# johannes-graeter/mono_lidar_depth

Measured on AMD Instinct MI355X. Metric: feature-depth associations/sec, higher is better.
Workload: dtype f64; 1 GPU; BASELINE config 2: 64x2048 cloud x 2000 features/frame, C0 parameters, 1024 HBM-resident frames/step/GPU; frame_slots_per_launch=1024, features_per_frame=2000, points_per_frame=131072, contexts=2, sequences=1, parallelism=sequence-per-gpu x1

## Files before the change

### mono_lidar_depth_amd/csrc/mld_api.hip

```cpp
#include <hip/hip_runtime.h>

#include <algorithm>

#include <cmath>
#include <cstdio>
#include <cstdlib>
#include <condition_variable>
#include <cstring>
#include <ctime>
#include <functional>
#include <limits>
#include <mutex>
#include <string>
#include <thread>
#include <vector>

#include "../../include/mld.h"
#include "mld_device.h"
#include "mld_kernels.hip"
#include "mld_ransac.hip"

using namespace mld;

namespace {
// ... 61 lines not shown
        }
    }
    void submit(std::function<int(std::string&)> j) {
        {
            std::lock_guard<std::mutex> lk(m);
            job = std::move(j);
            pending = true;
        }
        cv.notify_all();
    }
    int wait(std::string& e) {
        std::unique_lock<std::mutex> lk(m);
        cv.wait(lk, [&] { return !pending; });
        e = err;
        return rc;
    }
    void stop() {
        {
            std::lock_guard<std::mutex> lk(m);
            quit = true;
        }
        cv.notify_all();
        if (th.joinable()) th.join();
    }
};

struct ProjShare {
    hipStream_t stream = nullptr;
    int refs = 0;
};

struct mld_ctx {
    mld_params P{};
    mld_camera cam{};
    Calib calib{};
    int device = 0;
    hipStream_t stream = nullptr;
    bool own_stream = true;
    std::vector<Slot> slots;
    SlotDesc* d_slots = nullptr;
    unsigned char* dummy = nullptr;
    int32_t* queue_counts = nullptr;
    uint32_t* map_slab = nullptr;
    size_t map_stride = 0;
    int32_t* queue_slab = nullptr;
    uint32_t* bitmaps = nullptr;
    size_t bitmap_words = 0;
    std::vector<SlotDesc> h_descs;
    std::vector<SlotDesc> desc_stage;
    size_t lds_bytes = 0;
    size_t lds_fused = 0;
    size_t lds_classify = 0;
    bool classify_staged = true;
    int bm_ncol = 0, bm_ncolp = 0;
    bool force_thread_path = false;
    size_t proj_lds = 0;
    std::string err;
    int32_t* rs_flags = nullptr;
    int32_t* rs_cand = nullptr;
    int32_t* rs_block = nullptr;
    size_t rs_cap = 0;
    int32_t* rs_M = nullptr;
    int32_t* rs_S = nullptr;
    int32_t* rs_sample = nullptr;
    float* rs_sp = nullptr;
    int32_t* rs_counts = nullptr;
    size_t rs_counts_cap = 0;
    int32_t* rs_inl = nullptr;
    ransac::Result* rs_res = nullptr;
    unsigned char* sem_img = nullptr;
    size_t sem_img_cap = 0;
    float* sem_coeffs = nullptr;
    unsigned char* sem_groups = nullptr;
    size_t sem_groups_cap = 0;
    ransac::SemResult* sem_res = nullptr;
    double* trk_uv_cur = nullptr;
    double* trk_uv_last = nullptr;
    double* trk_depth_cur = nullptr;
    double* trk_depth_last = nullptr;
    int32_t* trk_type_cur = nullptr;
    int32_t* trk_type_last = nullptr;
    int32_t* trk_rank = nullptr;
    long long* trk_n_new = nullptr;
    size_t trk_cap = 0;
    unsigned char* trkb = nullptr;
    size_t trkb_cap = 0;
    int trkb_seqs = 0;
    TrkSeq* trkb_desc = nullptr;
    std::vector<TrkSeq> trkb_host;
    SlotDesc* d_sub = nullptr;
    int32_t* sub_counts = nullptr;
    size_t sub_cap = 0;
    std::vector<SlotDesc> h_sub;
    unsigned char* trk_stage = nullptr;
    size_t trk_stage_cap = 0;
    unsigned char* fr_host = nullptr;
    unsigned char* fr_dev = nullptr;
    size_t fr_cap = 0;
    unsigned char* fr_host_dev = nullptr;
    bool fr_zero_copy = true;
    bool fr_helper_on = true;
    hipEvent_t fr_ev[5] = {nullptr, nullptr, nullptr, nullptr, nullptr};
    double fr_us[10] = {0, 0, 0, 0, 0, 0, 0, 0, 0, 0};
    uint32_t* rsb_masks = nullptr;
    size_t rsb_mask_words = 0;
    PlaneDev* rsb_planes = nullptr;
// ... 186 lines not shown
    c.thrG_mode = P.treshold_depth_mode;
    c.thrG_min = (double)P.treshold_depth_min;
    c.thrG_max = (double)P.treshold_depth_max;
    c.thrL_en = P.treshold_depth_local_enabled;
    c.thrL_mode = P.treshold_depth_local_mode;
    c.thrL_type = P.treshold_depth_local_valuetype;
    c.thrL_val = P.treshold_depth_local_value;
    c.useTriMax = P.do_use_triangle_size_maximation;
    c.checkPlanar = P.do_check_triangleplanar_condition;
    c.planarThr = P.triangleplanar_crossnorm_treshold;
    c.orthThr = P.viewray_plane_orthoganality_treshold;
    c.cutBehind = P.do_use_cut_behind_camera;
    c.useRoad = P.do_use_ransac_plane;
    c.roadMode = P.plane_estimator_use_triangle_maximation ? 1 : 0;
    c.roadDistThr = P.ransac_plane_point_distance_treshold;
    c.roadDistThrF = (float)c.roadDistThr;
    c.padf2_ = 0.f;
    c.zxMinRel = P.plane_estimator_z_x_min_relation;
    c.usePCA = P.do_use_PCA;
    c.pcaAbsMin = P.pca_treshold_3_abs_min;
    c.pcaRelMax = P.pca_treshold_3_2_rel_max;
    c.pcaRelMin = P.pca_treshold_2_1_rel_min;
    ctx->lds_bytes = (size_t)cap * (3 * sizeof(double) + 2 * sizeof(int));
    c.threadPath = 1;
    c.xcdAware = 1;
    c.sortClasses = 4;
    c.k1max = 32;
    c.kMain = 24;
    c.kTotal = 40;
#ifdef MLD_AB_SWITCHES
    if (const char* e = std::getenv("MLD_FORCE_WAVE_PATH")) c.threadPath = (e[0] == '1') ? 0 : 1;
    if (const char* e = std::getenv("MLD_NO_XCD")) c.xcdAware = (e[0] == '1') ? 0 : 1;
    if (const char* e = std::getenv("MLD_SORT_CLASSES")) c.sortClasses = (e[0] == '4') ? 4 : 1;
    if (const char* e = std::getenv("MLD_FORCE_THREAD_PATH")) ctx->force_thread_path = e[0] == '1';
    if (const char* e = std::getenv("MLD_PROJ_LDS")) ctx->proj_lds = (size_t)std::atoll(e);
    if (const char* e = std::getenv("MLD_GATE")) ctx->gate_mode = e[0] != '0';
    if (const char* e = std::getenv("MLD_FRAME_COPY")) ctx->fr_zero_copy = e[0] != '1';
    if (const char* e = std::getenv("MLD_FRAME_HELPER")) ctx->fr_helper_on = e[0] != '0';
    if (const char* e = std::getenv("MLD_K1MAX")) c.k1max = std::min(std::max(std::atoi(e), 8), kK1MaxLimit);
    if (const char* e = std::getenv("MLD_KMAIN")) c.kMain = std::min(std::max(std::atoi(e), 8), c.k1max);
    if (std::getenv("MLD_K1MAX") || std::getenv("MLD_KMAIN")) c.kTotal = c.k1max + c.kMain;
    if (const char* e = std::getenv("MLD_KTOTAL")) c.kTotal = std::min(std::max(std::atoi(e), c.k1max), c.k1max + c.kMain);
#endif
    ctx->lds_fused = (size_t)c.kTotal * kWave * sizeof(uint32_t);
    ctx->bm_ncol = (ctx->cam.width + 31) / 32 + 1;
    ctx->bm_ncolp = ctx->bm_ncol | 1;
    const size_t cls_fixed = (size_t)(kClsBuckets + kClsThreads / kWave + 4) * sizeof(int);
    const size_t cls_bitmap = (size_t)c.bmStride * (size_t)ctx->bm_ncolp * sizeof(uint32_t);
    ctx->classify_staged = cls_fixed + cls_bitmap <= 128 * 1024;
#ifdef MLD_AB_SWITCHES
    if (const char* e = std::getenv("MLD_CLASSIFY_STAGED")) ctx->classify_staged = ctx->classify_staged && e[0] != '0';
#endif
    ctx->lds_classify = cls_fixed + (ctx->classify_staged ? cls_bitmap : 0);
}

hipStream_t projection_fork(mld_ctx* ctx, int& rc) {
    rc = MLD_OK;
    if (!ctx->proj_stream) return ctx->stream;
    hipError_t e = hipEventRecord(ctx->proj_fork, ctx->stream);
    if (e == hipSuccess) e = hipStreamWaitEvent(ctx->proj_stream, ctx->proj_fork, 0);
    if (e != hipSuccess) {
        ctx->err = std::string("projection stream (fork): ") + hipGetErrorString(e);
        rc = MLD_ERR_HIP;
    }
    return ctx->proj_stream;
}
int projection_join(mld_ctx* ctx) {
    if (!ctx->proj_stream) return MLD_OK;
    HIP_TRY(ctx, hipEventRecord(ctx->proj_join, ctx->proj_stream));
    HIP_TRY(ctx, hipStreamWaitEvent(ctx->stream, ctx->proj_join, 0));
    return MLD_OK;
}
struct ProjectionScope {
    mld_ctx* ctx;
    bool open = true;
    explicit ProjectionScope(mld_ctx* c) : ctx(c) {}
    int finish() {
        open = false;
        return projection_join(ctx);
    }
    ~ProjectionScope() {
        if (open && ctx->proj_stream) {
            const std::string keep = ctx->err;
            (void)projection_join(ctx);
            ctx->err = keep;
        }
    }
};

int enable_rs_batch_lds(mld_ctx* ctx, size_t lds) {
    static size_t enabled[64] = {};
    static std::mutex mtx;
    std::lock_guard<std::mutex> lk(mtx);
    size_t& cur = enabled[ctx->device & 63];
    if (lds <= cur) return MLD_OK;
    HIP_TRY(ctx, hipFuncSetAttribute(reinterpret_cast<const void*>(ransac::k_rs_batch),
                                     hipFuncAttributeMaxDynamicSharedMemorySize, (int)lds));
    cur = lds;
    return MLD_OK;
}

int check_slot(mld_ctx* ctx, int slot) {
    if (!ctx) return MLD_ERR_INVALID_ARG;
    if (slot < 0 || slot >= (int)ctx->slots.size()) return fail(ctx, MLD_ERR_INVALID_ARG, "slot out of range");
    return MLD_OK;
}
// ... 151 lines not shown
    }
    s.queues_in_slab = false;
    s.d.live_queue = nullptr;
    s.d.ovf_queue = nullptr;
    HIP_TRY(ctx, hipMalloc((void**)&s.d.ovf_queue, (size_t)F * 2 * sizeof(int32_t)));
    HIP_TRY(ctx, hipMalloc((void**)&s.d.live_queue, (size_t)F * sizeof(int32_t)));
    s.road_cap = (size_t)F;
    return MLD_OK;
}

int upload_descs(mld_ctx* ctx, int n_slots, hipStream_t st = nullptr, int first = 0, bool tags_in_descs = false);

int upload_small(mld_ctx* ctx, void* dst, const void* src, size_t bytes, hipStream_t st) {
    static_assert(sizeof(SlotDesc) % 4 == 0 && sizeof(TrkSeq) % 4 == 0 && sizeof(Calib) % 4 == 0, "k_upload moves 32-bit words");
    if (!bytes) return MLD_OK;
    if (bytes % 4) return fail(ctx, MLD_ERR_INVALID_ARG, "upload_small: size not a multiple of 4");
    if (bytes > ctx->up_gen_bytes) return fail(ctx, MLD_ERR_CAPACITY, "upload_small: table larger than the context's upload ring");
    const int g = ctx->up_next;
    if (ctx->up_busy[g]) HIP_TRY(ctx, hipEventSynchronize(ctx->up_ev[g]));
    if (!ctx->up_ev[g]) HIP_TRY(ctx, hipEventCreateWithFlags(&ctx->up_ev[g], hipEventDisableTiming));
    unsigned char* stage = ctx->up_base + (size_t)g * ctx->up_gen_bytes;
    std::memcpy(stage, src, bytes);
    const int words = (int)(bytes / 4);
    hipLaunchKernelGGL(mld::k_upload, dim3((unsigned)((words + 255) / 256)), dim3(256), 0, st, reinterpret_cast<uint32_t*>(dst),
                       reinterpret_cast<const uint32_t*>(stage), words);
    HIP_TRY(ctx, hipGetLastError());
    HIP_TRY(ctx, hipEventRecord(ctx->up_ev[g], st));
    ctx->up_busy[g] = true;
    ctx->up_next = (g + 1) % mld_ctx::kUpGens;
    return MLD_OK;
}

int launch_features(mld_ctx* ctx, int n_slots, int64_t max_F, bool single, int slot, const Calib* override_calib = nullptr,
                    const SlotDesc* group_descs = nullptr) {
    if (max_F <= 0) return MLD_OK;
    const SlotDesc* const descs = group_descs ? group_descs : ctx->d_slots;
    Calib calib = override_calib ? *override_calib : ctx->calib;
    const bool few = single && max_F <= 16384 && !ctx->force_thread_path;
    if (few) calib.threadPath = 0;
    const int per_slot = (int)((max_F + kWave - 1) / kWave);
    const uint32_t tag_all = (single || group_descs) ? 0u : common_tag(ctx, n_slots);
    const SlotDesc one = single ? ctx->slots[slot].d : SlotDesc{};
    const int use_single = single ? 1 : 0, ns = single ? 1 : n_slots;
    if (few) {
    } else {
        ScopedTimer ts(ctx, 5);
        auto kc = ctx->classify_staged ? mld::k_classify<true, kClsThreads, kClsKeep>
                                       : mld::k_classify<false, kClsThreads, kClsKeep>;
        const bool gate = ctx->gate_mode && ctx->release_waiter && !single;
        if (gate && !ctx->cls_done) {
            HIP_TRY(ctx, hipMalloc((void**)&ctx->cls_done, sizeof(uint32_t)));
            HIP_TRY(ctx, hipMemsetAsync(ctx->cls_done, 0, sizeof(uint32_t), ctx->stream));
        }
        hipLaunchKernelGGL(kc, dim3((unsigned)ns), dim3(kClsThreads), ctx->lds_classify, ctx->stream, descs, one,
                           use_single, calib, ctx->bm_ncol, ctx->bm_ncolp, gate ? ctx->cls_done : (uint32_t*)nullptr);
        if (gate) {
            mld_ctx* w = ctx->release_waiter;
            ctx->release_waiter = nullptr;
            w->waiting_on = nullptr;
            ctx->cls_target += (uint32_t)ns;
            if (w->gate_src && w->gate_src != ctx && w->gate_src->gate_waiter == w) w->gate_src->gate_waiter = nullptr;
            if (ctx->gate_waiter && ctx->gate_waiter != w) {
                ctx->gate_waiter->gate_counter = nullptr;
                ctx->gate_waiter->order_wait_pending = false;
                ctx->gate_waiter->gate_src = nullptr;
            }
            w->gate_counter = ctx->cls_done;
            w->gate_target = ctx->cls_target;
            w->order_wait_pending = true;
            w->gate_src = ctx;
            ctx->gate_waiter = w;
        }
    }
    if (ctx->release_waiter) {
        mld_ctx* w = ctx->release_waiter;
        ctx->release_waiter = nullptr;
        w->waiting_on = nullptr;
        HIP_TRY(ctx, hipEventRecord(w->order_ev, ctx->stream));
        if (w->gate_src && w->gate_src->gate_waiter == w) w->gate_src->gate_waiter = nullptr;
        w->gate_src = nullptr;
        w->gate_counter = nullptr;
        w->order_wait_pending = true;
    }
    int rc_up = MLD_OK;
    const Calib* d_calib = ctx->d_calib;
    {
        Calib want = calib;
        want.threadPath = ctx->calib.threadPath;
        const int which = std::memcmp(&want, &ctx->calib, sizeof(Calib)) == 0 ? 0 : 1;
        if (std::memcmp(&want, &ctx->calib_uploaded[which], sizeof(Calib)) != 0) {
            int rc_c = upload_small(ctx, ctx->d_calib + which, &want, sizeof(Calib), ctx->stream);
            if (rc_c) return rc_c;
            ctx->calib_uploaded[which] = want;
        }
        d_calib = ctx->d_calib + which;
    }
    if (calib.threadPath) {
        ScopedTimer tm(ctx, 1);
        int dense = (calib.k1max > 32 || calib.kMain > 24) ? ((ctx->shared_arg & 1) ? 1 : 2) : 0;
#ifdef MLD_AB_SWITCHES
        if (const char* e = std::getenv("MLD_FORCE_DENSE")) dense = std::min(std::max(std::atoi(e), 0), 2);
#endif
        auto kf = dense == 2 ? (calib.roadMode ? mld::k_feature_fused<1, 2> : mld::k_feature_fused<0, 2>)
                  : dense == 1 ? (calib.roadMode ? mld::k_feature_fused<1, 1> : mld::k_feature_fused<0, 1>)
                               : (calib.roadMode ? mld::k_feature_fused<1, 0> : mld::k_feature_fused<0, 0>);
        if (single && (rc_up = upload_descs(ctx, 1, nullptr, slot, true))) return rc_up;
        hipLaunchKernelGGL(kf, dim3((unsigned)per_slot * (unsigned)ns), dim3(kWave), ctx->lds_fused + ctx->lds_fused_pad, ctx->stream,
                           descs + (single ? slot : 0), d_calib, ns, per_slot);
    }
    {
        ScopedTimer tm(ctx, 3);
        const int chunk = few ? (int)std::min<int64_t>(8, std::max<int64_t>(1, (max_F + 8191) / 8192)) : 8;
        const int want = (int)((max_F + chunk - 1) / chunk);
// ... 169 lines not shown
        if (hipStreamCreateWithFlags(&fresh, hipStreamNonBlocking) != hipSuccess) break;
        rejected.push_back(ctx->stream);
        ctx->stream = fresh;
    }
    for (hipStream_t r : rejected) (void)hipStreamDestroy(r);
    g_live.push_back(ctx);
}
}

mld_ctx* mld_create(const mld_params* params, const mld_camera* camera, const double T_cam_lidar[12], int device,
                    int max_frames, int64_t max_points, int64_t max_features, int* status_out) {
    auto bail = [&](int code, const std::string& msg) -> mld_ctx* {
        g_create_error = msg;
        if (status_out) *status_out = code;
        return nullptr;
    };
    if (status_out) *status_out = MLD_OK;
    if (!params || !camera || !T_cam_lidar) return bail(MLD_ERR_INVALID_ARG, "null argument");
    if (max_frames < 1) return bail(MLD_ERR_INVALID_ARG, "max_frames must be >= 1");
    if (camera->width < 1 || camera->height < 1) return bail(MLD_ERR_INVALID_ARG, "bad image size");
    if (camera->width > 65535 || camera->height > 65535 || (int64_t)camera->width * camera->height > (int64_t)1 << 30)
        return bail(MLD_ERR_CAPACITY, "image larger than 65535 pixels on a side or 2^30 pixels in all");
    if (!std::isfinite(camera->focal_length) || camera->focal_length == 0.0 || !std::isfinite(camera->principal_point_x) ||
        !std::isfinite(camera->principal_point_y))
        return bail(MLD_ERR_INVALID_ARG, "bad camera intrinsics");
    for (int t = 0; t < 12; t++)
        if (!std::isfinite(T_cam_lidar[t])) return bail(MLD_ERR_INVALID_ARG, "non-finite lidar->camera transform");
    if (max_points > kMaxPoints) return bail(MLD_ERR_CAPACITY, "max_points exceeds 8 388 607");
    std::string why;
    int v = validate_params(*params, why);
    if (v != MLD_OK) return bail(v, why);

    int ndev = 0;
    hipError_t e = hipGetDeviceCount(&ndev);
    if (e != hipSuccess || ndev < 1)
        return bail(MLD_ERR_HIP, std::string("no HIP device available (") + hipGetErrorString(e) +
                                     "): the DepthEstimator path has no CPU fallback");
    if (device < 0 || device >= ndev) return bail(MLD_ERR_INVALID_ARG, "device index out of range");

    mld_ctx* ctx = new mld_ctx();
    ctx->P = *params;
    ctx->cam = *camera;
    ctx->device = device;
    build_calib(ctx, T_cam_lidar);
    auto hip_bail = [&](hipError_t err, const char* what) -> mld_ctx* {
        std::string m = std::string(what) + ": " + hipGetErrorString(err);
        mld_destroy(ctx);
        return bail(MLD_ERR_HIP, m);
    };
    if ((e = hipSetDevice(device)) != hipSuccess) return hip_bail(e, "hipSetDevice");
    hipDeviceProp_t prop;
    if ((e = hipGetDeviceProperties(&prop, device)) != hipSuccess) return hip_bail(e, "hipGetDeviceProperties");
    ctx->lds_per_cu = (size_t)prop.maxSharedMemoryPerMultiProcessor;
    if (ctx->lds_bytes > (size_t)prop.sharedMemPerBlock) {
        mld_destroy(ctx);
        return bail(MLD_ERR_CAPACITY, "search window too large for the LDS-staged neighbour list");
    }
    if ((e = hipStreamCreateWithFlags(&ctx->stream, hipStreamNonBlocking)) != hipSuccess)
        return hip_bail(e, "hipStreamCreate");
    separate_stream_from_live_contexts(ctx);
    if (ctx->lds_bytes > 48 * 1024) {
        e = hipFuncSetAttribute(reinterpret_cast<const void*>(mld::k_feature_wave<true>), hipFuncAttributeMaxDynamicSharedMemorySize,
                                (int)ctx->lds_bytes);
        if (e == hipSuccess)
            e = hipFuncSetAttribute(reinterpret_cast<const void*>(mld::k_feature_wave<false>),
                                    hipFuncAttributeMaxDynamicSharedMemorySize, (int)ctx->lds_bytes);
        if (e != hipSuccess) return hip_bail(e, "hipFuncSetAttribute(k_feature_wave)");
    }
    if (ctx->lds_classify > 48 * 1024) {
        e = hipFuncSetAttribute(reinterpret_cast<const void*>(mld::k_classify<true, kClsThreads, kClsKeep>),
                                hipFuncAttributeMaxDynamicSharedMemorySize, (int)ctx->lds_classify);

        if (e != hipSuccess) return hip_bail(e, "hipFuncSetAttribute(k_classify)");
    }
    if (ctx->lds_fused > 48 * 1024) {
        const void* fused[] = {reinterpret_cast<const void*>(mld::k_feature_fused<0, 0>),
                               reinterpret_cast<const void*>(mld::k_feature_fused<1, 0>),
                               reinterpret_cast<const void*>(mld::k_feature_fused<0, 1>),
                               reinterpret_cast<const void*>(mld::k_feature_fused<1, 1>),
                               reinterpret_cast<const void*>(mld::k_feature_fused<0, 2>),
                               reinterpret_cast<const void*>(mld::k_feature_fused<1, 2>)};
        for (const void* f : fused) {
            e = hipFuncSetAttribute(f, hipFuncAttributeMaxDynamicSharedMemorySize, (int)ctx->lds_fused);
            if (e != hipSuccess) return hip_bail(e, "hipFuncSetAttribute(k_feature_fused)");
        }
    }
    ctx->slots.resize(max_frames);
    ctx->h_descs.resize(max_frames);
    if ((e = hipMalloc((void**)&ctx->d_slots, sizeof(SlotDesc) * max_frames)) != hipSuccess)
        return hip_bail(e, "hipMalloc(slots)");
    if ((e = hipMalloc((void**)&ctx->dummy, 256)) != hipSuccess) return hip_bail(e, "hipMalloc(dummy)");
    if ((e = hipMalloc((void**)&ctx->d_calib, 2 * sizeof(Calib))) != hipSuccess) return hip_bail(e, "hipMalloc(calib)");
    std::memset(ctx->calib_uploaded, 0xFF, sizeof(ctx->calib_uploaded));
    constexpr size_t kMaxGroupDescs = 256;
    static_assert(kMaxGroupDescs <= 512, "the group descriptors of a launch set must fit one generation of the upload ring");
    static_assert(sizeof(TrkSeq) <= 2 * sizeof(SlotDesc), "a sequence's TrkSeq must fit the ring share of its two slots");
    const size_t up_descs = max_frames >= 2 ? std::max<size_t>((size_t)max_frames, 512) : 1;
    ctx->up_gen_bytes = (std::max(sizeof(SlotDesc) * up_descs, sizeof(Calib)) + 4095) / 4096 * 4096;
    if ((e = hipHostMalloc((void**)&ctx->up_base, ctx->up_gen_bytes * mld_ctx::kUpGens, hipHostMallocDefault)) != hipSuccess)
        return hip_bail(e, "hipHostMalloc(upload ring)");
    if ((e = hipMemsetAsync(ctx->dummy, 0, 256, ctx->stream)) != hipSuccess) return hip_bail(e, "hipMemset(dummy)");
    size_t cells = (size_t)camera->width * camera->height + kMapPadCells;
    ctx->bitmap_words = (size_t)ctx->calib.bmStride * (size_t)((camera->width + 31) / 32 + 1) + 4;
    const size_t cnt_words = 2 * (size_t)max_frames;
    if ((e = hipMalloc((void**)&ctx->queue_counts, (cnt_words + ctx->bitmap_words * (size_t)max_frames) * sizeof(uint32_t))) != hipSuccess)
        return hip_bail(e, "hipMalloc(bitmaps)");
    ctx->bitmaps = reinterpret_cast<uint32_t*>(ctx->queue_counts) + cnt_words;
    if ((e = hipMemsetAsync(ctx->queue_counts, 0, cnt_words * sizeof(uint32_t), ctx->stream)) != hipSuccess)
        return hip_bail(e, "hipMemset(counters)");
    for (size_t si = 0; si < ctx->slots.size(); si++) ctx->slots[si].d.bitmap = ctx->bitmaps + si * ctx->bitmap_words;
    for (size_t si = 0; si < ctx->slots.size(); si++) {
        ctx->slots[si].d.live_count = ctx->queue_counts + si;
        ctx->slots[si].d.ovf_count = ctx->queue_counts + (size_t)max_frames + si;
    }
    const size_t map_stride = (cells + 63) & ~(size_t)63;
    ctx->map_stride = map_stride;
    if ((e = hipMalloc((void**)&ctx->map_slab, map_stride * (size_t)max_frames * sizeof(uint32_t))) != hipSuccess)
        return hip_bail(e, "hipMalloc(maps)");
    if ((e = hipMemsetAsync(ctx->map_slab, 0, map_stride * (size_t)max_frames * sizeof(uint32_t), ctx->stream)) != hipSuccess)
        return hip_bail(e, "hipMemset(maps)");
    const size_t qF = max_features > 0 ? (((size_t)max_features + 63) & ~(size_t)63) : 0;
    const size_t q_stride = qF * 3;
    if (qF && (e = hipMalloc((void**)&ctx->queue_slab, q_stride * (size_t)max_frames * sizeof(int32_t))) != hipSuccess)
        return hip_bail(e, "hipMalloc(queues)");
    for (size_t si = 0; si < ctx->slots.size(); si++) {
        Slot& s = ctx->slots[si];
// ... 1745 lines not shown
```

### mono_lidar_depth_amd/csrc/mld_kernels.hip

```cpp
#include "mld_device.h"
#include "../../include/mld.h"
#include "mld_diag.h"

namespace mld {

#define GPTR(T, p) ((const T __attribute__((address_space(1)))*)(p))
#define GPTRW(T, p) ((T __attribute__((address_space(1)))*)(p))
#define CPTR(T, p) ((const T __attribute__((address_space(4)))*)(p))
typedef float f32x4 __attribute__((ext_vector_type(4)));
typedef uint32_t u32x4u __attribute__((ext_vector_type(4), aligned(4)));

__device__ __forceinline__ int prefix_count(unsigned long long m) {
    return (int)__builtin_amdgcn_mbcnt_hi((unsigned)(m >> 32), __builtin_amdgcn_mbcnt_lo((unsigned)m, 0u));
}
__device__ __forceinline__ int uniform(int v) { return __builtin_amdgcn_readfirstlane(v); }
__device__ __forceinline__ bool wave_any(bool p) { return __builtin_amdgcn_ballot_w64(p) != 0ull; }
__device__ __forceinline__ double readlane_f64(double v, int lane) {
    int lo = __double2loint(v), hi = __double2hiint(v);
    lo = __builtin_amdgcn_readlane(lo, lane);
    hi = __builtin_amdgcn_readlane(hi, lane);
    return __hiloint2double(hi, lo);
}
template <int CTRL, int ROW_MASK>
__device__ __forceinline__ int dpp_self(int v) {
// ... 2045 lines not shown
                }
            const double mx = sx / (double)n, my = sy / (double)n, mz = sz / (double)n;
            double c0 = 0, c1 = 0, c2 = 0, c3 = 0, c4 = 0, c5 = 0;
            for (int e = 0; e < nmax; e++)
                if (e < n) {
                    V3 p = cam_point(c, s, LST(e));
                    double dx = p.x - mx, dy = p.y - my, dz = p.z - mz;
                    c0 += dx * dx;
                    c1 += dx * dy;
                    c2 += dx * dz;
                    c3 += dy * dy;
                    c4 += dy * dz;
                    c5 += dz * dz;
                }
            r[0] = mx; r[1] = my; r[2] = mz;
            r[3] = c0; r[4] = c1; r[5] = c2; r[6] = c3; r[7] = c4; r[8] = c5;
        } else if (live) {
            V3 p0 = cam_point(c, s, LST(0)), p1 = cam_point(c, s, LST(1)), p2 = cam_point(c, s, LST(2));
            r[0] = p0.x; r[1] = p0.y; r[2] = p0.z;
            r[3] = p1.x; r[4] = p1.y; r[5] = p1.z;
            r[6] = p2.x; r[7] = p2.y; r[8] = p2.z;
        }
    }
    r[9] = minZ;
    r[10] = maxZ;
    ST_USE_F64(r[0]);
    ST_USE_F64(r[8]);
    ST_MARK(10);
    if (live) finish_main(c, pca, myu, myv, r, mytype, mydepth);
    ST_USE_F64(mydepth);
    ST_MARK(11);
}

template <int DENSE>
__device__ __forceinline__ void main_after_scan(const Calib& c, const SlotRef& s, uint32_t* lst, const int lane,
                                                const int lcap, const int k, bool live, const double myu, const double myv,
                                                int& mytype, double& mydepth, bool& overflow ST_ARG) {
    int ks;
    double minZ, maxZ;
    const int kmax0 = uniform(wave_max_i32(live ? k : 0));
    if (DENSE && kmax0 > kZcDefault && (kmax0 <= kZcMid || DENSE == 1))
        main_hist<DENSE ? kZcMid : kZcDefault>(c, s, lst, lane, lcap, k, live, mytype, ks, minZ, maxZ ST_PASS);
    else if (DENSE == 2 && kmax0 > kZcMid)
        main_hist<DENSE == 2 ? kZcDense : kZcDefault>(c, s, lst, lane, lcap, k, live, mytype, ks, minZ, maxZ ST_PASS);
    else if (DENSE == 0 && kmax0 <= kZcTiny)
        main_hist<DENSE == 0 ? kZcTiny : kZcDefault>(c, s, lst, lane, lcap, k, live, mytype, ks, minZ, maxZ ST_PASS);
    else if (DENSE == 0 && kmax0 <= kZcShort)
        main_hist<DENSE == 0 ? kZcShort : kZcDefault>(c, s, lst, lane, lcap, k, live, mytype, ks, minZ, maxZ ST_PASS);
    else
        main_hist<kZcDefault>(c, s, lst, lane, lcap, k, live, mytype, ks, minZ, maxZ ST_PASS);
    main_tail<DENSE>(c, s, lst, lane, lcap, ks, live, minZ, maxZ, myu, myv, mytype, mydepth, overflow ST_PASS);
}

template <bool DIRECT>
__global__ __launch_bounds__(kWave) void k_feature_wave(const SlotDesc* __restrict__ slots, SlotDesc single, int use_single,
                                                        const Calib* __restrict__ calib, int n_slots, int per_slot,
                                                        uint32_t tag_all, int chunk) {
    constexpr int direct = DIRECT ? 1 : 0;
    const Calib& c = *calib;
    extern __shared__ __align__(16) unsigned char smem[];
    int slot, j;
    decode_block((int)blockIdx.x, c.xcdAware ? n_slots : -n_slots, per_slot, slot, j);
    SlotDesc s = use_single ? single : slots[slot];
    apply_plane_dev(s);
    if (tag_all) s.tag = tag_all;
    int count;
    if (direct) {
        long long Fn = s.F;
        if (s.F_dev) {
            long long fd = *GPTR(long long, s.F_dev) - s.F_dev_off;
            fd = fd < 0 ? 0 : fd;
            Fn = fd < Fn ? fd : Fn;
        }
        count = (int)Fn;
    } else {
        if (!s.ovf_count) return;
        count = *GPTR(int32_t, s.ovf_count);
    }
    const int lane = threadIdx.x;
    auto pass = [&](const int e0) {
        bool active = lane < chunk && e0 + lane < count;
        long long f = 0;
        int code = 0;
        double myu = 0, myv = 0;
        if (active && direct) {
            f = e0 + lane;
            code = -1;
            const auto* q = GPTR(double, s.uv) + 2 * f;
            myu = q[0];
            myv = q[1];
            int x0, y0, nx, ny;
            if (window_bounds(c, myu, myv, c.halfX1, c.halfY1, x0, y0, nx, ny) && nx <= 32) {
                const auto* bm = GPTR(uint32_t, s.bitmap) + (size_t)(x0 >> 5) * (size_t)c.bmStride;
                const uint32_t sh = (uint32_t)(x0 & 31);
                const uint32_t colmask = (nx >= 32) ? ~0u : ((1u << nx) - 1u);
                int k1 = 0;
                for (int r = 0; r < ny; r++) {
                    const uint32_t lo = bm[y0 + r], hi = bm[c.bmStride + y0 + r];
                    k1 += __popc(__builtin_amdgcn_alignbit(hi, lo, sh) & colmask);
                }
                if ((unsigned)k1 < c.countMin) {
                    GPTRW(double, s.depth)[f] = -1.0;
                    if (s.type) GPTRW(int32_t, s.type)[f] = MLD_RadiusSearchInsufficientPoints;
                    active = false;
                }
            } else if (nx <= 32) {
                if (0u < c.countMin) {
                    GPTRW(double, s.depth)[f] = -1.0;
                    if (s.type) GPTRW(int32_t, s.type)[f] = MLD_RadiusSearchInsufficientPoints;
                    active = false;
                }
            }
        } else if (active) {
            f = (long long)GPTR(int32_t, s.ovf_queue)[2 * (size_t)(e0 + lane)];
            code = GPTR(int32_t, s.ovf_queue)[2 * (size_t)(e0 + lane) + 1];
            const auto* q = GPTR(double, s.uv) + 2 * f;
            myu = q[0];
            myv = q[1];
        }
        int mytype = code < 0 ? (int)MLD_Unspecified : code;
        double mydepth = -1.0;
        const unsigned long long all = __ballot(active);
        const unsigned long long full = __ballot(active && code < 0);
        double corners[9];
        bool has_corners = false;
        ST_BEGIN(1);
        wave_path(c, s, smem, lane, all, myu, myv, mytype, mydepth, full, corners, has_corners ST_PASS);
        if (active) {
            GPTRW(double, s.depth)[f] = mydepth;
            if (s.type) GPTRW(int32_t, s.type)[f] = mytype;
            if (s.corners && has_corners) {
#pragma unroll
                for (int t = 0; t < 9; t++) GPTRW(double, s.corners)[9 * f + t] = corners[t];
            }
        }
        ST_MARK(12);
        ST_END();
    };
    if (DIRECT) {
        if (j * chunk < count) pass(j * chunk);
    } else {
        for (int e0 = j * chunk; e0 < count; e0 += per_slot * chunk) pass(e0);
    }
}


__device__ __forceinline__ bool window_bounds(const Calib& c, double u, double v, double halfX, double halfY, int& x0,
                                              int& y0, int& nx, int& ny) {
    x0 = 0;
    y0 = 0;
    nx = 0;
    ny = 0;
    if (!(isfinite(u) && isfinite(v))) return false;
    double a;
    a = u - halfX;
    const double left = (a < 0.) ? 0. : a;
    a = u + halfX;
    const double right = ((double)(c.W - 1) < a) ? (double)(c.W - 1) : a;
    a = v - halfY;
    const double top = (a < 0.) ? 0. : a;
    a = v + halfY;
    const double bottom = ((double)(c.H - 1) < a) ? (double)(c.H - 1) : a;
    const int xa = (int)left, ya = (int)top, xb = (int)right, yb = (int)bottom;
    const int wx = xb - xa + 1, wy = yb - ya + 1;
    if (wx <= 0 || wy <= 0 || xa < 0 || ya < 0 || xb >= c.W || yb >= c.H) return false;
    x0 = xa;
    y0 = ya;
    nx = wx;
    ny = wy;
    return true;
}

constexpr int kClsThreads = 1024;
constexpr int kClsBuckets = 1024;
constexpr int kClsKeep = 2;
enum : int { CLS_DEAD = -1, CLS_OVF = -2, CLS_NONE = -3 };

template <bool STAGED, int kClsThreads, int kClsKeep>
__global__ __launch_bounds__(kClsThreads) void k_classify(const SlotDesc* __restrict__ slots, SlotDesc single,
                                                          int use_single, Calib c, int ncol, int ncolp,
                                                          uint32_t* __restrict__ done) {
    extern __shared__ __align__(16) unsigned char smem[];
    int* hist = reinterpret_cast<int*>(smem);
    int* wsum = hist + kClsBuckets;
    int* ctr = wsum + kClsThreads / kWave;
    uint32_t* lbm = reinterpret_cast<uint32_t*>(ctr + 4);
    SlotDesc s = use_single ? single : slots[blockIdx.x];
    apply_plane_dev(s);
    long long Fn = s.F;
    if (s.F_dev) {
        long long fd = *GPTR(long long, s.F_dev) - s.F_dev_off;
        fd = fd < 0 ? 0 : fd;
        Fn = fd < Fn ? fd : Fn;
    }
    const int tid = threadIdx.x, lane = tid & (kWave - 1), wave = tid >> 6;
// ... 105 lines not shown
                fu[q] = uv[2 * i];
                fv[q] = uv[2 * i + 1];
            }
        }
#pragma unroll
        for (int q = 0; q < kClsKeep; q++) {
            const long long i = tid + (long long)q * kClsThreads;
            kept[q] = (i < Fn) ? classify(fu[q], fv[q]) : (int)CLS_NONE;
            if (kept[q] >= 0) atomicAdd(&hist[kept[q]], 1);
            if (i < Fn) settle(i, kept[q]);
        }
    }
    for (long long i = tid + (long long)kClsKeep * kClsThreads; i < Fn; i += kClsThreads) {
        const int cls = classify(uv[2 * i], uv[2 * i + 1]);
        if (cls >= 0) atomicAdd(&hist[cls], 1);
        settle(i, cls);
    }
    __syncthreads();
    constexpr int kPer = kClsBuckets / kClsThreads;
    static_assert(kPer >= 1 && kPer * kClsThreads == kClsBuckets, "bucket count must be a multiple of the block size");
    int loc[kPer], sum = 0;
#pragma unroll
    for (int q = 0; q < kPer; q++) {
        loc[q] = hist[tid * kPer + q];
        sum += loc[q];
    }
    int incl = sum;
#pragma unroll
    for (int d = 1; d < kWave; d <<= 1) {
        const int t = __shfl_up(incl, d);
        if (lane >= d) incl += t;
    }
    if (lane == kWave - 1) wsum[wave] = incl;
    __syncthreads();
    int base = incl - sum;
    for (int q = 0; q < wave; q++) base += wsum[q];
    if (tid == kClsThreads - 1) {
        *GPTRW(int32_t, s.live_count) = base + sum;
        *GPTRW(int32_t, s.ovf_count) = ctr[0];
    }
#pragma unroll
    for (int q = 0; q < kPer; q++) {
        hist[tid * kPer + q] = base;
        base += loc[q];
    }
    __syncthreads();
    auto* live = GPTRW(int32_t, s.live_queue);
#pragma unroll
    for (int q = 0; q < kClsKeep; q++)
        if (kept[q] >= 0) live[atomicAdd(&hist[kept[q]], 1)] = (int32_t)(tid + q * kClsThreads);
    for (long long i = tid + (long long)kClsKeep * kClsThreads; i < Fn; i += kClsThreads) {
        const int cls = classify(uv[2 * i], uv[2 * i + 1]);
        if (cls >= 0) live[atomicAdd(&hist[cls], 1)] = (int32_t)i;
    }
}

__global__ __launch_bounds__(kWave) void k_gate(const uint32_t* __restrict__ counter, uint32_t target, int max_polls) {
    if (threadIdx.x != 0) return;
    for (int i = 0; i < max_polls; i++) {
        const uint32_t v = __hip_atomic_load(GPTR(uint32_t, counter), __ATOMIC_RELAXED, __HIP_MEMORY_SCOPE_AGENT);
        if ((int32_t)(v - target) >= 0) break;
        __builtin_amdgcn_s_sleep(32);
    }
}

__global__ __launch_bounds__(kWave) void k_probe_wait(const uint32_t* flag, uint32_t* result, int max_polls) {
    if (threadIdx.x != 0) return;
    uint32_t seen = 2u;
    for (int i = 0; i < max_polls; i++) {
        if (__hip_atomic_load(flag, __ATOMIC_RELAXED, __HIP_MEMORY_SCOPE_SYSTEM) != 0u) {
            seen = 1u;
            break;
        }
        __builtin_amdgcn_s_sleep(32);
    }
    __hip_atomic_store(result, seen, __ATOMIC_RELAXED, __HIP_MEMORY_SCOPE_SYSTEM);
}
__global__ void k_probe_set(uint32_t* flag) {
    if (threadIdx.x == 0 && blockIdx.x == 0) __hip_atomic_store(flag, 1u, __ATOMIC_RELAXED, __HIP_MEMORY_SCOPE_SYSTEM);
}

__global__ __launch_bounds__(256) void k_upload(uint32_t* __restrict__ dst, const uint32_t* __restrict__ src_host, int n_words) {
    const int i = blockIdx.x * 256 + threadIdx.x;
    if (i < n_words) dst[i] = __builtin_nontemporal_load(src_host + i);
}

#ifndef MLD_KEY_BATCH_F
#define MLD_KEY_BATCH_F 8
#endif
constexpr int kKeyBatchF = MLD_KEY_BATCH_F;
#ifndef MLD_DENSE_BATCH_MUL
#define MLD_DENSE_BATCH_MUL 2
#endif
constexpr int kDenseBatchMul = MLD_DENSE_BATCH_MUL;

template <int KB>
__device__ __forceinline__ int scan_window_flagged(const Calib& c, const SlotRef& s, int x0, int y0, int nx, int ny,
                                                   int xn0, int yn0, int nxn, int nyn, uint32_t* lst,
                                                   int lane, int& kflag, uint32_t& states, int& nbase, int& nroom ST_ARG) {
    const int nymax = uniform(wave_max_i32(ny));
    const auto* bm = GPTR(uint32_t, s.g.bitmap);
    const uint32_t colmask = (nx >= 32) ? ~0u : ((1u << nx) - 1u);
    const uint32_t nmask = (nxn > 0) ? (((nxn >= 32) ? ~0u : ((1u << nxn) - 1u)) << (xn0 - x0)) : 0u;
    int k = 0, kf = 0;
    const auto* col0 = bm + (size_t)(x0 >> 5) * (size_t)c.bmStride + (size_t)y0;
    const auto* col1 = col0 + c.bmStride;
// ... 448 lines not shown
```

Baseline: 2.833 billion feature-depth associations/s.

## Add persistent prefetching classify kernel and deal overflow work across waves

Adds k_classify_resident, a grid-limited persistent classify kernel. Each block loops over frame slots and prefetches the next slot's bitmap and uv data into registers while finishing the current one. It is only used when MLD_CLASSIFY_GRID is set, because the default grid value of -1 disables it. Separately, the overflow pass of k_feature_wave now spreads overflow entries across all waves with a stride instead of giving each wave a contiguous chunk. This balances lightly loaded slots at the cost of less coalesced queue reads.

```diff
diff --git a/mono_lidar_depth_amd/csrc/mld_api.hip b/mono_lidar_depth_amd/csrc/mld_api.hip
--- a/mono_lidar_depth_amd/csrc/mld_api.hip
+++ b/mono_lidar_depth_amd/csrc/mld_api.hip
@@ -137,6 +137,9 @@
     size_t lds_fused = 0;
     size_t lds_classify = 0;
     bool classify_staged = true;
+    size_t lds_classify_res = 0;
+    int cls_grid = kClsGridDefault;
+    int cu_count = 0;
     int bm_ncol = 0, bm_ncolp = 0;
     bool force_thread_path = false;
     size_t proj_lds = 0;
@@ -429,6 +432,7 @@
     if (const char* e = std::getenv("MLD_CLASSIFY_STAGED")) ctx->classify_staged = ctx->classify_staged && e[0] != '0';
 #endif
     ctx->lds_classify = cls_fixed + (ctx->classify_staged ? cls_bitmap : 0);
+    ctx->lds_classify_res = std::max(ctx->lds_classify, kClsResidentLds);
 }
 
 hipStream_t projection_fork(mld_ctx* ctx, int& rc) {
@@ -686,13 +690,20 @@
             HIP_TRY(ctx, hipMalloc((void**)&ctx->cls_done, sizeof(uint32_t)));
             HIP_TRY(ctx, hipMemsetAsync(ctx->cls_done, 0, sizeof(uint32_t), ctx->stream));
         }
-        hipLaunchKernelGGL(kc, dim3((unsigned)ns), dim3(kClsThreads), ctx->lds_classify, ctx->stream, descs, one,
-                           use_single, calib, ctx->bm_ncol, ctx->bm_ncolp, gate ? ctx->cls_done : (uint32_t*)nullptr);
+        const bool resident = !single && ctx->classify_staged && ctx->cls_grid >= 0 && ctx->cu_count > 0;
+        const int grid = !resident ? ns : std::min(ns, ctx->cls_grid > 0 ? ctx->cls_grid : ctx->cu_count);
+        if (resident)
+            hipLaunchKernelGGL(mld::k_classify_resident, dim3((unsigned)grid), dim3(kClsThreads), ctx->lds_classify_res,
+                               ctx->stream, descs, calib, ctx->bm_ncol, ctx->bm_ncolp, ns,
+                               gate ? ctx->cls_done : (uint32_t*)nullptr);
+        else
+            hipLaunchKernelGGL(kc, dim3((unsigned)ns), dim3(kClsThreads), ctx->lds_classify, ctx->stream, descs, one,
+                               use_single, calib, ctx->bm_ncol, ctx->bm_ncolp, gate ? ctx->cls_done : (uint32_t*)nullptr);
         if (gate) {
             mld_ctx* w = ctx->release_waiter;
             ctx->release_waiter = nullptr;
             w->waiting_on = nullptr;
-            ctx->cls_target += (uint32_t)ns;
+            ctx->cls_target += (uint32_t)grid;
             if (w->gate_src && w->gate_src != ctx && w->gate_src->gate_waiter == w) w->gate_src->gate_waiter = nullptr;
             if (ctx->gate_waiter && ctx->gate_waiter != w) {
                 ctx->gate_waiter->gate_counter = nullptr;
@@ -968,6 +979,8 @@
     hipDeviceProp_t prop;
     if ((e = hipGetDeviceProperties(&prop, device)) != hipSuccess) return hip_bail(e, "hipGetDeviceProperties");
     ctx->lds_per_cu = (size_t)prop.maxSharedMemoryPerMultiProcessor;
+    ctx->cu_count = prop.multiProcessorCount;
+    if (const char* e = std::getenv("MLD_CLASSIFY_GRID")) ctx->cls_grid = std::max(std::atoi(e), -1);
     if (ctx->lds_bytes > (size_t)prop.sharedMemPerBlock) {
         mld_destroy(ctx);
         return bail(MLD_ERR_CAPACITY, "search window too large for the LDS-staged neighbour list");
@@ -988,6 +1001,12 @@
                                 hipFuncAttributeMaxDynamicSharedMemorySize, (int)ctx->lds_classify);
 
         if (e != hipSuccess) return hip_bail(e, "hipFuncSetAttribute(k_classify)");
+    }
+    if (!ctx->classify_staged || ctx->lds_classify_res > ctx->lds_per_cu) ctx->cls_grid = -1;
+    if (ctx->cls_grid >= 0) {
+        e = hipFuncSetAttribute(reinterpret_cast<const void*>(mld::k_classify_resident),
+                                hipFuncAttributeMaxDynamicSharedMemorySize, (int)ctx->lds_classify_res);
+        if (e != hipSuccess) return hip_bail(e, "hipFuncSetAttribute(k_classify_resident)");
     }
     if (ctx->lds_fused > 48 * 1024) {
         const void* fused[] = {reinterpret_cast<const void*>(mld::k_feature_fused<0, 0>),
diff --git a/mono_lidar_depth_amd/csrc/mld_kernels.hip b/mono_lidar_depth_amd/csrc/mld_kernels.hip
--- a/mono_lidar_depth_amd/csrc/mld_kernels.hip
+++ b/mono_lidar_depth_amd/csrc/mld_kernels.hip
@@ -2121,6 +2121,10 @@
     main_tail<DENSE>(c, s, lst, lane, lcap, ks, live, minZ, maxZ, myu, myv, mytype, mydepth, overflow ST_PASS);
 }
 
+#ifndef MLD_WAVE_DEAL
+#define MLD_WAVE_DEAL 1
+#endif
+constexpr bool kWaveDeal = MLD_WAVE_DEAL != 0;
 template <bool DIRECT>
 __global__ __launch_bounds__(kWave) void k_feature_wave(const SlotDesc* __restrict__ slots, SlotDesc single, int use_single,
                                                         const Calib* __restrict__ calib, int n_slots, int per_slot,
@@ -2147,13 +2151,14 @@
         count = *GPTR(int32_t, s.ovf_count);
     }
     const int lane = threadIdx.x;
-    auto pass = [&](const int e0) {
-        bool active = lane < chunk && e0 + lane < count;
+    auto pass = [&](const int e0, const int estride) {
+        const int e = e0 + lane * estride;
+        bool active = lane < chunk && e < count;
         long long f = 0;
         int code = 0;
         double myu = 0, myv = 0;
         if (active && direct) {
-            f = e0 + lane;
+            f = e;
             code = -1;
             const auto* q = GPTR(double, s.uv) + 2 * f;
             myu = q[0];
@@ -2181,8 +2186,8 @@
                 }
             }
         } else if (active) {
-            f = (long long)GPTR(int32_t, s.ovf_queue)[2 * (size_t)(e0 + lane)];
-            code = GPTR(int32_t, s.ovf_queue)[2 * (size_t)(e0 + lane) + 1];
+            f = (long long)GPTR(int32_t, s.ovf_queue)[2 * (size_t)e];
+            code = GPTR(int32_t, s.ovf_queue)[2 * (size_t)e + 1];
             const auto* q = GPTR(double, s.uv) + 2 * f;
             myu = q[0];
             myv = q[1];
@@ -2207,9 +2212,12 @@
         ST_END();
     };
     if (DIRECT) {
-        if (j * chunk < count) pass(j * chunk);
+        if (j * chunk < count) pass(j * chunk, 1);
     } else {
-        for (int e0 = j * chunk; e0 < count; e0 += per_slot * chunk) pass(e0);
+        const bool deal = kWaveDeal && count <= per_slot * chunk;
+        const int first = deal ? j : j * chunk, step = deal ? count : per_slot * chunk;
+        const int end = deal ? (count < per_slot ? count : per_slot) : count;
+        for (int e0 = first; e0 < end; e0 += step) pass(e0, deal ? per_slot : 1);
     }
 }
 
@@ -2421,6 +2429,257 @@
     for (long long i = tid + (long long)kClsKeep * kClsThreads; i < Fn; i += kClsThreads) {
         const int cls = classify(uv[2 * i], uv[2 * i + 1]);
         if (cls >= 0) live[atomicAdd(&hist[cls], 1)] = (int32_t)i;
+    }
+}
+
+constexpr int kClsResStage = 4;
+constexpr int kClsGridDefault = -1;
+constexpr size_t kClsResidentLds = 82 * 1024;
+struct ClsAhead {
+    const uint32_t* bitmap;
+    const double* uv;
+    long long F;
+    const long long* f_dev;
+    const int* has_plane;
+};
+struct ClsSlot {
+    const uint32_t* bitmap;
+    const double* uv;
+    double* depth;
+    int32_t* type;
+    int32_t* ovf_queue;
+    int32_t* ovf_count;
+    int32_t* live_queue;
+    int32_t* live_count;
+    long long F, f_dev_off;
+    bool mask;
+};
+__device__ __forceinline__ ClsAhead cls_ahead(const SlotDesc* __restrict__ slots, int i) {
+    const auto* d = CPTR(SlotDesc, slots + i);
+    ClsAhead r;
+    r.bitmap = d->bitmap;
+    r.uv = d->uv;
+    r.F = d->F;
+    const long long* fdev = d->F_dev;
+    const PlaneDev* pdv = d->plane_dev;
+    r.f_dev = fdev ? fdev : &slots[i].F;
+    r.has_plane = pdv ? &pdv->has_plane : &slots[i].has_plane;
+    return r;
+}
+__device__ __forceinline__ ClsSlot cls_slot(const SlotDesc* __restrict__ slots, int i) {
+    const auto* d = CPTR(SlotDesc, slots + i);
+    ClsSlot r;
+    r.bitmap = d->bitmap;
+    r.uv = d->uv;
+    r.depth = d->depth;
+    r.type = d->type;
+    r.ovf_queue = d->ovf_queue;
+    r.ovf_count = d->ovf_count;
+    r.live_queue = d->live_queue;
+    r.live_count = d->live_count;
+    r.F = d->F;
+    const long long off = d->F_dev_off;
+    r.f_dev_off = d->F_dev ? off : 0;
+    r.mask = d->inlier_mask != nullptr;
+    return r;
+}
+__global__ __launch_bounds__(kClsThreads, 5) void k_classify_resident(const SlotDesc* __restrict__ slots, Calib c, int ncol,
+                                                                   int ncolp, int n_slots, uint32_t* __restrict__ done) {
+    extern __shared__ __align__(16) unsigned char smem[];
+    int* hist = reinterpret_cast<int*>(smem);
+    int* wsum = hist + kClsBuckets;
+    int* ctr = wsum + kClsThreads / kWave;
+    uint32_t* lbm = reinterpret_cast<uint32_t*>(ctr + 4);
+    const int tid = threadIdx.x, lane = tid & (kWave - 1), wave = tid >> 6;
+    int si = (int)blockIdx.x;
+    if (si >= n_slots) return;
+    if (done && tid == 0) __hip_atomic_fetch_add(GPTRW(uint32_t, done), 1u, __ATOMIC_RELAXED, __HIP_MEMORY_SCOPE_AGENT);
+    const int stepG = (int)gridDim.x;
+    const int q4 = c.bmStride >> 2, n4 = ncol * q4;
+    const int rot = (lane >> 3) & 3;
+    const float rq = 1.0f / (float)q4;
+    auto piece = [&](int t, int& col, int& y) -> bool {
+        int tv = tid;
+        asm volatile("" : "+v"(tv));
+        const int g = tv + t * kClsThreads;
+        col = (int)(((float)g + 0.5f) * rq);
+        y = (g - col * q4) << 2;
+        return g < n4;
+    };
+    u32x4u pw[kClsResStage];
+    double pu[kClsKeep], pvv[kClsKeep];
+    long long pfd;
+    int php;
+    int vzero = 0;
+    asm volatile("" : "+v"(vzero));
+    auto fetch = [&](const ClsAhead& d) {
+        const auto* bm = GPTR(uint32_t, d.bitmap);
+#pragma unroll
+        for (int t = 0; t < kClsResStage; t++) {
+            int col, y;
+            const int off = piece(t, col, y) ? col * c.bmStride + y : 0;
+            pw[t] = *GPTR(u32x4u, bm + off);
+        }
+        const bool any = d.F > 0 && d.uv;
+        const auto* uv = any ? GPTR(double, d.uv) : GPTR(double, &slots[0]);
+        const long long last = any ? d.F - 1 : 0;
+#pragma unroll
+        for (int q = 0; q < kClsKeep; q++) {
+            long long i = tid + (long long)q * kClsThreads;
+            i = i < last ? i : last;
+            pu[q] = uv[2 * i];
+            pvv[q] = uv[2 * i + 1];
+        }
+        pfd = GPTR(long long, d.f_dev)[vzero];
+        php = GPTR(int, d.has_plane)[vzero];
+    };
+    fetch(cls_ahead(slots, si));
+    ClsAhead a1 = cls_ahead(slots, si + stepG < n_slots ? si + stepG : si);
+    const int rowBuckets = c.sortClasses > 1 ? kClsBuckets / 4 : kClsBuckets;
+    const double scale = (double)rowBuckets / (double)c.H;
+    for (;;) {
+        const ClsSlot s = cls_slot(slots, si);
+        for (int b = tid; b < kClsBuckets; b += kClsThreads) hist[b] = 0;
+        if (tid == 0) ctr[0] = 0;
+#pragma unroll
+        for (int t = 0; t < kClsResStage; t++) {
+            u32x4u w = pw[t];
+            if (rot & 1) w = u32x4u{w[1], w[2], w[3], w[0]};
+            if (rot & 2) w = u32x4u{w[2], w[3], w[0], w[1]};
+            int col, y;
+            if (piece(t, col, y)) {
+#pragma unroll
+                for (int k = 0; k < 4; k++) lbm[(y + ((k + rot) & 3)) * ncolp + col] = w[k];
+            }
+        }
+        double fu[kClsKeep], fv[kClsKeep];
+#pragma unroll
+        for (int q = 0; q < kClsKeep; q++) {
+            fu[q] = pu[q];
+            fv[q] = pvv[q];
+        }
+        long long Fn = s.F;
+        {
+            long long fd = pfd - s.f_dev_off;
+            fd = fd < 0 ? 0 : fd;
+            Fn = fd < Fn ? fd : Fn;
+        }
+        const bool road_on = c.useRoad && php && s.mask;
+        const auto* bm = GPTR(uint32_t, s.bitmap);
+        for (int g0 = tid + kClsResStage * kClsThreads; g0 < n4; g0 += kClsThreads) {
+            const int col = (int)(((float)g0 + 0.5f) * rq), y = (g0 - col * q4) << 2;
+            const u32x4u w = *GPTR(u32x4u, bm + (size_t)col * c.bmStride + y);
+#pragma unroll
+            for (int k = 0; k < 4; k++) lbm[(y + k) * ncolp + col] = w[k];
+        }
+        const int sn = si + stepG;
+        fetch(a1);
+        const int sn2 = sn + stepG;
+        a1 = cls_ahead(slots, sn2 < n_slots ? sn2 : (sn < n_slots ? sn : si));
+        __syncthreads();
+        const auto* uv = GPTR(double, s.uv);
+        auto count_window = [&](int x0, int y0, int nx, int ny) -> int {
+            const int cx = x0 >> 5, sh = x0 & 31;
+            const uint32_t colmask = (nx >= 32) ? ~0u : ((1u << nx) - 1u);
+            int k = 0;
+            for (int r = 0; r < ny; r++) {
+                const int y = y0 + r;
+                const uint32_t lo = lbm[y * ncolp + cx], hi = lbm[y * ncolp + cx + 1];
+                k += __popc(__builtin_amdgcn_alignbit(hi, lo, (uint32_t)sh) & colmask);
+            }
+            return k;
+        };
+        auto classify = [&](double u, double v) -> int {
+            int x0, y0, nx, ny;
+            int k1 = 0;
+            if (window_bounds(c, u, v, c.halfX1, c.halfY1, x0, y0, nx, ny)) {
+                if (nx > 32) return CLS_OVF;
+                k1 = count_window(x0, y0, nx, ny);
+                if (!c.threadPath) return ((unsigned)k1 < c.countMin) ? (int)CLS_DEAD : (int)CLS_OVF;
+                if (road_on) {
+                    int a0, a1, anx, any_;
+                    if (window_bounds(c, u, v, c.halfX2, c.halfY2, a0, a1, anx, any_) && anx > 32) return CLS_OVF;
+                }
+                if (k1 > c.kMain || k1 > c.kTotal) return CLS_OVF;
+                if (road_on && (3 * k1 > c.k1max || 4 * k1 > c.kTotal)) {
+                    int a0, a1, anx, any_;
+                    if (window_bounds(c, u, v, c.halfX2, c.halfY2, a0, a1, anx, any_)) {
+                        const int k2 = count_window(a0, a1, anx, any_);
+                        if (k2 > c.k1max || k1 + k2 > c.kTotal) return CLS_OVF;
+                    }
+                }
+            }
+            if ((unsigned)k1 < c.countMin) return CLS_DEAD;
+            if (!c.threadPath) return CLS_OVF;
+            int b = 0;
+            if (v > 0.0) b = (v < (double)c.H) ? (int)(v * scale) : rowBuckets - 1;
+            b = b < rowBuckets ? b : rowBuckets - 1;
+            const int cls = (k1 <= 8) ? 0 : ((k1 <= 12) ? 1 : ((k1 <= 16) ? 2 : 3));
+            return (c.sortClasses > 1 ? (3 - cls) * rowBuckets : 0) + b;
+        };
+        auto settle = [&](long long i, int cls) {
+            if (cls == CLS_DEAD) {
+                GPTRW(double, s.depth)[i] = -1.0;
+                if (s.type) GPTRW(int32_t, s.type)[i] = MLD_RadiusSearchInsufficientPoints;
+            } else if (cls == CLS_OVF) {
+                const int pos = atomicAdd(&ctr[0], 1);
+                GPTRW(int32_t, s.ovf_queue)[2 * (size_t)pos] = (int32_t)i;
+                GPTRW(int32_t, s.ovf_queue)[2 * (size_t)pos + 1] = -1;
+            }
+        };
+        int kept[kClsKeep];
+#pragma unroll
+        for (int q = 0; q < kClsKeep; q++) {
+            const long long i = tid + (long long)q * kClsThreads;
+            kept[q] = (i < Fn) ? classify(fu[q], fv[q]) : (int)CLS_NONE;
+            if (kept[q] >= 0) atomicAdd(&hist[kept[q]], 1);
+            if (i < Fn) settle(i, kept[q]);
+        }
+        for (long long i = tid + (long long)kClsKeep * kClsThreads; i < Fn; i += kClsThreads) {
+            const int cls = classify(uv[2 * i], uv[2 * i + 1]);
+            if (cls >= 0) atomicAdd(&hist[cls], 1);
+            settle(i, cls);
+        }
+        __syncthreads();
+        constexpr int kPer = kClsBuckets / kClsThreads;
+        static_assert(kPer >= 1 && kPer * kClsThreads == kClsBuckets, "bucket count must be a multiple of the block size");
+        int loc[kPer], sum = 0;
+#pragma unroll
+        for (int q = 0; q < kPer; q++) {
+            loc[q] = hist[tid * kPer + q];
+            sum += loc[q];
+        }
+        int incl = sum;
+#pragma unroll
+        for (int d = 1; d < kWave; d <<= 1) {
+            const int t = __shfl_up(incl, d);
+            if (lane >= d) incl += t;
+        }
+        if (lane == kWave - 1) wsum[wave] = incl;
+        __syncthreads();
+        int base = incl - sum;
+        for (int q = 0; q < wave; q++) base += wsum[q];
+        if (tid == kClsThreads - 1) {
+            *GPTRW(int32_t, s.live_count) = base + sum;
+            *GPTRW(int32_t, s.ovf_count) = ctr[0];
+        }
+#pragma unroll
+        for (int q = 0; q < kPer; q++) {
+            hist[tid * kPer + q] = base;
+            base += loc[q];
+        }
+        __syncthreads();
+        auto* live = GPTRW(int32_t, s.live_queue);
+#pragma unroll
+        for (int q = 0; q < kClsKeep; q++)
+            if (kept[q] >= 0) live[atomicAdd(&hist[kept[q]], 1)] = (int32_t)(tid + q * kClsThreads);
+        for (long long i = tid + (long long)kClsKeep * kClsThreads; i < Fn; i += kClsThreads) {
+            const int cls = classify(uv[2 * i], uv[2 * i + 1]);
+            if (cls >= 0) live[atomicAdd(&hist[cls], 1)] = (int32_t)i;
+        }
+        if (sn >= n_slots) break;
+        si = sn;
+        __syncthreads();
     }
 }
 
```

After: 2.834 billion feature-depth associations/s, median of 2. No clear change (+0.0%).
